# leaxer-ai/leaxer-qwen3-tts

Measured on AMD Instinct MI355X. Metric: real-time factor (24 kHz audio sec / wall sec), Qwen3-TTS-0.6B, higher is better.
Workload: dtype bf16 weights, fp32 activations/accumulate (codec decoder: fp16 hi/lo split operands, fp32 accumulate)

## Files before the change

### leaxer-qwen3-tts_amd/csrc/q3_codec.cpp

```cpp
#include <algorithm>
#include <cmath>
#include <cstdlib>
#include <cstring>
#include <unordered_map>
#include <vector>

#include "q3_engine.h"

namespace q3 {

struct PackedConv { const float* w = nullptr; const float* b = nullptr; int cin = 0, cout = 0, k = 0; };
struct SnakeP { const float *alpha = nullptr, *beta = nullptr; int C = 0; };

struct CodecW {
    struct Layer { const float *in_norm, *post_norm, *qkv, *o, *gate, *up, *down, *attn_scale, *mlp_scale; };
    std::vector<Layer> layers;
    const float *norm = nullptr, *code_embed = nullptr;
    struct Up { PackedConv tconv; const float *dw_w, *dw_b, *ln_w, *ln_b, *pw1_w, *pw1_b, *pw2_w, *pw2_b, *gamma; };
    std::vector<Up> up;
    PackedConv conv_in, conv_out;
    struct Res { SnakeP a1, a2; PackedConv c1, c2; };
    struct Block { SnakeP act; PackedConv tconv; Res res[3]; };
    std::vector<Block> blocks;
    SnakeP snake_out;
// ... 246 lines not shown
        auto take = [&](size_t nfloat) -> float* {
            const size_t bytes = (nfloat * sizeof(float) + 255) & ~(size_t)255;
            float* p = plan ? nullptr : (float*)(W.arena[lane] + off);
            off += bytes;
            return p;
        };
        const size_t kslab_floats = (size_t)32 * 128 * 4096;
        float* kslab = take(kslab_floats);
        auto conv = [&](ConvArgs a) {
            if (plan) return;
            a.slab = kslab; a.slab_floats = kslab_floats; a.batch = nbatch;
            const auto it = W.planes.find(a.W);
            if (it != W.planes.end()) { a.Wh = it->second.hi; a.Wl = it->second.lo; a.Whc = it->second.cm; a.w_scale_inv = it->second.scale_inv; a.w_lo_zero = it->second.lo_zero; }
            if (a.snake_alpha) { const auto sp = W.snake_pre.find(a.snake_alpha); if (sp != W.snake_pre.end()) a.snake_pre = sp->second; }
            if (a.mid_alpha) { const auto sp = W.snake_pre.find(a.mid_alpha); if (sp != W.snake_pre.end()) a.mid_pre = sp->second; }
            launch_conv(a, stream);
        };
        auto gemm = [&](const float* in, int T, int Cin, const float* Wm, const float* bias, int Cout, float* out) {
            ConvArgs a; a.in = in; a.T_in = T; a.C_in = Cin; a.out = out; a.T_out = T; a.C_out = Cout; a.W = Wm; a.bias = bias;
            return a;
        };
        float* h = take((size_t)F * CH);
        float* hn = take((size_t)F * CH);
        float* qkvb = take((size_t)F * 3 * CH);
        float* att = take((size_t)F * CH);
        float* ub = take((size_t)F * FF);
        float* gb = take((size_t)F * FF);
        float* kc = take((size_t)NH * P * HD);
        float* vc = take((size_t)NH * P * HD);
        if (!plan && !h_in) launch_code_embed_mean(W.code_embed, codes_dev, F, c.n_groups, c.cd_codebook, CH, h, stream);
        for (int l = 0; l < (h_in ? 0 : c.cd_layers); ++l) {
            const CodecW::Layer& L = W.layers[l];
            if (!plan) launch_rmsnorm_rows(h, L.in_norm, c.cd_rms_eps, F, CH, hn, stream);
// ... 35 lines not shown
        }
        const bool fp32_act = knob("Q3TTS_CONV_FP32_ACT") != nullptr || knob("Q3TTS_CONV_GENERIC_EPILOGUE") != nullptr;
        bool act_planes = !fp32_act && !W.planes.empty() && CH % 32 == 0 && W.planes.count(W.conv_in.w) && !W.snake_pre.empty();
        for (int i = 0, Cw = D; i <= c.cd_n_blocks; ++i, Cw /= 2) act_planes = act_planes && Cw % 96 == 0;
        for (const CodecW::Block& B : W.blocks) {
            act_planes = act_planes && W.planes.count(B.tconv.w);
            for (int u = 0; u < 3; ++u) act_planes = act_planes && W.planes.count(B.res[u].c1.w) && W.planes.count(B.res[u].c2.w);
        }
        float* x = take(nbz * Tc * D);
        float* sx = take(nbz * Tc * D);
        { ConvArgs a; a.in = cur; a.T_in = Tc; a.C_in = CH; a.out = x; a.T_out = Tc; a.C_out = D; a.W = W.conv_in.w; a.bias = W.conv_in.b; a.taps = 7;
          a.in_ustride = nbatch > 1 ? h_ustride : 0;
          a.out2 = sx; a.snake_alpha = W.blocks[0].act.alpha; a.snake_beta = W.blocks[0].act.beta; a.out2_planes = act_planes; conv(a); }
        int C = D;
        static const int dil[3] = { 1, 3, 9 };
        for (int i = 0; i < c.cd_n_blocks; ++i) {
            const CodecW::Block& B = W.blocks[i];
            const int r = c.cd_up_rates[i], Co = C / 2;
            int left = 0;
            const int To = tconv_out_len(c, Tc, 2 * r, r, &left);
            float* nx = take(nbz * To * Co);
            float* ns = take(nbz * To * Co);
            float* nt = take(nbz * To * Co);
            { ConvArgs a; a.in = sx; a.T_in = Tc; a.C_in = C; a.out = nx; a.T_out = To; a.C_out = Co; a.W = B.tconv.w; a.bias = B.tconv.b;
              a.taps = 2 * r; a.transposed = 1; a.stride = r; a.left = left; a.in_planes = act_planes;
              a.out2 = ns; a.snake_alpha = B.res[0].a1.alpha; a.snake_beta = B.res[0].a1.beta; a.out2_planes = act_planes; conv(a); }
            for (int u = 0; u < 3; ++u) {
                const CodecW::Res& R = B.res[u];
                const SnakeP nxt = u < 2 ? B.res[u + 1].a1 : (i + 1 < c.cd_n_blocks ? W.blocks[i + 1].act : W.snake_out);
                const bool nxt_planes = act_planes && !(u == 2 && i + 1 == c.cd_n_blocks);
                const auto p2 = W.planes.find(R.c2.w);
                if (Co == 96 && p2 != W.planes.end() && W.planes.count(R.c1.w) && !knob("Q3TTS_NO_FUSED_RES")) {
                    ConvArgs a; a.in = ns; a.T_in = To; a.C_in = Co; a.out = nx; a.T_out = To; a.C_out = Co; a.W = R.c1.w; a.bias = R.c1.b;
                    a.taps = 7; a.dil = dil[u]; a.mid_alpha = R.a2.alpha; a.mid_beta = R.a2.beta;
                    a.W2 = R.c2.w; a.W2h = p2->second.hi; a.W2l = p2->second.lo; a.W2fh = p2->second.fh; a.W2fl = p2->second.fl; a.w2_scale_inv = p2->second.scale_inv; a.w2_lo_zero = p2->second.lo_zero; a.bias2 = R.c2.b;
// ... 2 lines not shown
                    conv(a);
                    std::swap(ns, nt);
                    continue;
                }
                { ConvArgs a; a.in = ns; a.T_in = To; a.C_in = Co; a.out = nullptr; a.T_out = To; a.C_out = Co; a.W = R.c1.w; a.bias = R.c1.b;
                  a.taps = 7; a.dil = dil[u]; a.out2 = nt; a.snake_alpha = R.a2.alpha; a.snake_beta = R.a2.beta;
                  a.in_planes = act_planes; a.out2_planes = act_planes; conv(a); }
                { ConvArgs a; a.in = nt; a.T_in = To; a.C_in = Co; a.out = nx; a.T_out = To; a.C_out = Co; a.W = R.c2.w; a.bias = R.c2.b;
                  a.taps = 1; a.res = nx; a.out2 = ns; a.snake_alpha = nxt.alpha; a.snake_beta = nxt.beta;
                  a.in_planes = act_planes; a.out2_planes = nxt_planes; conv(a); }
            }
            x = nx; sx = ns; Tc = To; C = Co;
        }
        pcm = take(nbz * Tc);
        { ConvArgs a; a.in = sx; a.T_in = Tc; a.C_in = C; a.out = pcm; a.T_out = Tc; a.C_out = 1; a.W = W.conv_out.w; a.bias = W.conv_out.b;
          a.taps = 7; a.clamp = 1; conv(a); }
        if (!plan && nbatch > 1) { W.dbg_sx = sx; W.dbg_pcm = pcm; W.dbg_T = Tc; W.dbg_C = C; W.dbg_nb = nbatch; }
        n_pcm = Tc;
        if (plan && off > W.arena_bytes[lane]) {
            Q3_HIP_CHECK(hipStreamSynchronize(stream));
            if (W.arena[lane]) (void)hipFree(W.arena[lane]);
            W.arena[lane] = nullptr;
            Q3_HIP_CHECK(hipMalloc((void**)&W.arena[lane], off));
            W.arena_bytes[lane] = off;
        }
    }
    *pcm_dev = pcm;
    return n_pcm;
}


// ... 1128 lines not shown
```

### leaxer-qwen3-tts_amd/csrc/q3_codec_kernels.hip

```cpp
#include <cstdlib>
#include <type_traits>
#include <utility>

#include "q3_common.h"

namespace q3 {

typedef float f32x16 __attribute__((ext_vector_type(16)));

#ifdef Q3_SAMPLE_PROF
__device__ long long g_conv_prof[64];
void conv_prof_read(long long* out) { (void)hipMemcpyFromSymbol(out, HIP_SYMBOL(g_conv_prof), sizeof(long long) * 64); }
#ifndef Q3_CONV_PROF_SEL
#define Q3_CONV_PROF_SEL (a.taps == 1 && a.C_in == 3072 && a.C_out == 1024)
#endif
#ifndef Q3_CONV_PROF_WG
#define Q3_CONV_PROF_WG 0
#endif
#define CP_MARK_IF(k, lim) do { __builtin_amdgcn_sched_barrier(0); \
        if ((k) < (lim) && blockIdx.x == Q3_CONV_PROF_WG && blockIdx.y == 0 && blockIdx.z == 0 && threadIdx.x == 0 && (Q3_CONV_PROF_SEL)) g_conv_prof[k] = wall_clock64(); \
        __builtin_amdgcn_sched_barrier(0); } while (0)
#define CP_MARK(k) CP_MARK_IF(k, 64)
#define CP_MARK_L(k) CP_MARK_IF(k, 46)
#else
// ... 32 lines not shown
    int act, clamp;
    float* out2; const float* s2_alpha; const float* s2_beta;
    const bf16_t* Wh; const bf16_t* Wl;
    float acc_scale;
    int ksplit; float* slab;
    int xcd_map;
    int no_fast_epi;
    int peel_taps;
    int in_planes, out2_planes;
    const float* s2_pre; const float* s1_pre;
    int batch_tiles;
    size_t in_ustride;
    const bf16_t* W2h; const bf16_t* W2l; float acc_scale2; const float* bias2; const float* s1_alpha; const float* s1_beta;
    int wlo;
    const bf16_t* W2fh; const bf16_t* W2fl;
};

static __device__ __forceinline__ void conv_tile_ids(bool remap, int& bx, int& by, int& bz) {
    bx = blockIdx.x; by = blockIdx.y; bz = blockIdx.z;
    const int nx = gridDim.x, ny = gridDim.y, nyz = ny * gridDim.z;
    if (!remap || nyz == 1) return;
    const int L = bx + nx * (by + ny * bz), gsz = 8 * nyz, full = nx >> 3;
    int G = L / gsz, w = 8;
    if (G >= full) { G = full; w = nx & 7; }
    const int r = L - G * gsz;
    bx = G * 8 + r % w;
    const int yz = r / w;
    by = yz % ny; bz = yz / ny;
}

// ... 88 lines not shown

typedef _Float16 f16x8 __attribute__((ext_vector_type(8)));
typedef _Float16 f16x4 __attribute__((ext_vector_type(4)));
#define B3_LD 40

typedef _Float16 f16x2 __attribute__((ext_vector_type(2)));
typedef float f32x2 __attribute__((ext_vector_type(2)));
static __device__ __forceinline__ void split_f16x2(float a, float b, f16x2& hi, f16x2& lo) {
    const f32x2 c = { __builtin_amdgcn_fmed3f(a, -65504.f, 65504.f), __builtin_amdgcn_fmed3f(b, -65504.f, 65504.f) };
    hi = __builtin_convertvector(c, f16x2);
    const f32x2 back = __builtin_convertvector(hi, f32x2);
    const f32x2 r = { __builtin_amdgcn_fmed3f(a - back.x, -65504.f, 65504.f), __builtin_amdgcn_fmed3f(b - back.y, -65504.f, 65504.f) };
    lo = __builtin_convertvector(r, f16x2);
}
__device__ float g_conv_dump[2][64 * 4];
template <int NB, bool OUT, bool RES, int RH, bool O2P = false>
static __device__ __forceinline__ void split_epilogue_snake(const ConvKArgs& a, const f32x16 (&acc)[NB], float* stage, int mrow0, int co0w,
                                                            int lane, int phase, int NT) {
    constexpr int W = NB * 32, LDE = W + 8;
    const int c4 = lane & 31, rsel = lane >> 5;
    const int co = co0w + c4 * 4;
    const bool colok = c4 * 4 < W && co < a.C_out;
    const int coc = colok ? co : 0, lc = c4 * 4 < W ? c4 * 4 : 0;
    const int m0r = mrow0 + rsel;
    const int t0 = a.transposed ? m0r * a.stride + phase - a.left : m0r, tstep = a.transposed ? 2 * a.stride : 2;
    const int mlim = a.transposed ? a.T_in + NT - 1 : 0x7fffffff;
    auto row_ok = [&](int p) { const int t = t0 + p * tstep; return colok && t >= 0 && t < a.T_out && m0r + 2 * p < mlim; };
    auto row_off = [&](int p) -> size_t { return row_ok(p) ? (size_t)(t0 + p * tstep) * a.C_out + coc : (size_t)coc; };
    float4 resv[RH];
    auto load_res = [&](int slot0, int p0, int n) {
#pragma unroll
        for (int k = 0; k < n; ++k) resv[slot0 + k] = *reinterpret_cast<const float4*>(a.res + row_off(p0 + k));
    };
    if (RES) load_res(0, 0, RH);
    const float4 bias4 = *reinterpret_cast<const float4*>(a.bias + coc);
    const float4 ea4 = *reinterpret_cast<const float4*>(a.s2_pre + coc), ib4 = *reinterpret_cast<const float4*>(a.s2_pre + a.C_out + coc);
#pragma unroll
    for (int j = 0; j < NB; ++j)
#pragma unroll
        for (int reg = 0; reg < 16; ++reg) stage[((reg & 3) + 8 * (reg >> 2) + 4 * rsel) * LDE + j * 32 + c4] = acc[j][reg];
    const float ea[4] = { ea4.x, ea4.y, ea4.z, ea4.w }, ib[4] = { ib4.x, ib4.y, ib4.z, ib4.w };
    const float bs[4] = { bias4.x, bias4.y, bias4.z, bias4.w };
    float* const dump1 = &g_conv_dump[0][lane * 4];
    float* const dump2 = &g_conv_dump[1][lane * 4];
#pragma unroll
    for (int p = 0; p < 16; ++p) {
        const bool okp = row_ok(p);
        const size_t o = row_off(p);
        const float4 raw = *reinterpret_cast<const float4*>(&stage[(p * 2 + rsel) * LDE + lc]);
        float v[4] = { raw.x, raw.y, raw.z, raw.w }, s2[4];
        const float4 r4 = RES ? resv[p % RH] : make_float4(0.f, 0.f, 0.f, 0.f);
        const float rv[4] = { r4.x, r4.y, r4.z, r4.w };
#pragma unroll
        for (int e = 0; e < 4; ++e) {
            float x = v[e] * a.acc_scale + bs[e];
            if (RES) x = rv[e] + x;
            v[e] = x;
            s2[e] = x + ib[e] * sin_sq(x * ea[e]);
        }
        if (OUT) *reinterpret_cast<float4*>(okp ? a.out + o : dump1) = make_float4(v[0], v[1], v[2], v[3]);
        if (O2P) {
            f16x2 h01, h23, l01, l23;
            split_f16x2(s2[0], s2[1], h01, l01);
            split_f16x2(s2[2], s2[3], h23, l23);
            *reinterpret_cast<uint4*>(okp ? a.out2 + o : dump2) =
                make_uint4(__builtin_bit_cast(unsigned, h01), __builtin_bit_cast(unsigned, h23), __builtin_bit_cast(unsigned, l01), __builtin_bit_cast(unsigned, l23));
        } else
        *reinterpret_cast<float4*>(okp ? a.out2 + o : dump2) = make_float4(s2[0], s2[1], s2[2], s2[3]);
        if ((p & 3) == 3) {
            __builtin_amdgcn_sched_barrier(0);
            if (RES && RH == 8 && p < 8) load_res(p - 3, p + 5, 4);
            __builtin_amdgcn_sched_barrier(0);
        }
    }
}

template <int NB, int RH = 16>
static __device__ __forceinline__ void split_epilogue_block(const ConvKArgs& a, const f32x16 (&acc)[NB], float* stage, int mrow0, int co0w,
                                                            int lane, int phase, int NT) {
    if (a.out2 && a.s2_pre && a.bias && a.act == 0 && !a.mul && !a.res_scale && !a.no_fast_epi) {
        if (a.out2_planes) {
            if (a.res) { if (a.out) split_epilogue_snake<NB, true, true, RH, true>(a, acc, stage, mrow0, co0w, lane, phase, NT);
                         else split_epilogue_snake<NB, false, true, RH, true>(a, acc, stage, mrow0, co0w, lane, phase, NT); }
            else { if (a.out) split_epilogue_snake<NB, true, false, RH, true>(a, acc, stage, mrow0, co0w, lane, phase, NT);
                   else split_epilogue_snake<NB, false, false, RH, true>(a, acc, stage, mrow0, co0w, lane, phase, NT); }
            return;
        }
        if (a.res) { if (a.out) split_epilogue_snake<NB, true, true, RH>(a, acc, stage, mrow0, co0w, lane, phase, NT);
                     else split_epilogue_snake<NB, false, true, RH>(a, acc, stage, mrow0, co0w, lane, phase, NT); }
        else { if (a.out) split_epilogue_snake<NB, true, false, RH>(a, acc, stage, mrow0, co0w, lane, phase, NT);
               else split_epilogue_snake<NB, false, false, RH>(a, acc, stage, mrow0, co0w, lane, phase, NT); }
        return;
    }
    constexpr int W = NB * 32, LDE = W + 8;
// ... 61 lines not shown
                }
                if (okp) {
                    if (a.out) *reinterpret_cast<float4*>(a.out + o) = make_float4(v[0], v[1], v[2], v[3]);
                    if (OUT2) *reinterpret_cast<float4*>(a.out2 + o) = make_float4(s2[0], s2[1], s2[2], s2[3]);
                }
            }
#pragma unroll
            for (int k = 0; k < 4; ++k) { resv[k] = resn[k]; mulv[k] = muln[k]; }
        }
    };
    using I0 = std::integral_constant<int, 0>; using I1 = std::integral_constant<int, 1>; using I2 = std::integral_constant<int, 2>;
    if (a.out2) { if (a.act == 0) rows(I0{}, std::true_type{}); else if (a.act == 1) rows(I1{}, std::true_type{}); else rows(I2{}, std::true_type{}); }
    else { if (a.act == 0) rows(I0{}, std::false_type{}); else if (a.act == 1) rows(I1{}, std::false_type{}); else rows(I2{}, std::false_type{}); }
}

template <int MB, int NB, int WM, int WN, int PA, int KC = 32, int NBUF = 2, bool F2 = false, bool PEEL = false, bool APL = false, bool WLO = true>
__global__ __launch_bounds__(256) __attribute__((amdgpu_waves_per_eu((MB * NB <= 6 && KC == 32 ? 2 : 1), (MB * NB <= 6 && KC == 32 ? 2 : 1))))
void k_conv_split(ConvKArgs a0) {
    ConvKArgs a = a0;
    int bx, by, bz;
    conv_tile_ids(a.xcd_map != 0, bx, by, bz);
    bx = conv_batch_rebase(a, bx);
    constexpr int TM = WM * MB * 32, TN = WN * NB * 32, AROWS = PA * 32;
    constexpr int CB = KC / 32, SEG = KC / 8, LD = KC + 8;
    constexpr int BPL = WLO ? 2 : 1, PBT = TN * SEG * BPL;
    constexpr int PB = (PBT + 255) / 256;
    constexpr int A_BYTES = 2 * AROWS * LD * 2, B_BYTES = NBUF * 2 * TN * LD * 2;
    constexpr int E_BYTES = 4 * 32 * (NB * 32 + 8) * 4;
    constexpr int SM_BYTES = A_BYTES + B_BYTES > E_BYTES ? A_BYTES + B_BYTES : E_BYTES;
    __shared__ __attribute__((aligned(16))) unsigned char smem[SM_BYTES];
    _Float16 (*As)[AROWS][LD] = reinterpret_cast<_Float16 (*)[AROWS][LD]>(smem);
// ... 16 lines not shown
        for (int j = 0; j < NB; ++j) acc[i][j] = zero16;

    const int arow = tid >> 3, acol = (tid & 7) * 4;
    typedef unsigned u32x4 __attribute__((ext_vector_type(4)));
    typedef float f32x4v __attribute__((ext_vector_type(4)));
    f32x4v areg[PA][CB];
    u32x4 breg[PB];
    const char* const in_bytes = reinterpret_cast<const char*>(a.in);
    unsigned aoff[PA];
#pragma unroll
    for (int i = 0; i < PA; ++i) {
        const int src = m0 - halo + arow + 32 * i;
        const int sc = src < 0 ? 0 : (src < a.T_in ? src : a.T_in - 1);
        aoff[i] = ((unsigned)sc * (unsigned)a.C_in + (unsigned)acol) * 4u;
    }
    auto loadA = [&](int ci0) {
        const char* const base = in_bytes + (size_t)ci0 * 4;
#pragma unroll
        for (int i = 0; i < PA; ++i)
#pragma unroll
            for (int cb = 0; cb < CB; ++cb) areg[i][cb] = *reinterpret_cast<const f32x4v*>(base + cb * 128 + aoff[i]);
    };
    const char* const w_bytes = reinterpret_cast<const char*>(a.Wh);
    const unsigned w_lo = (unsigned)(reinterpret_cast<const char*>(a.Wl) - reinterpret_cast<const char*>(a.Wh));
    constexpr bool w_cm = KC == 32;
    const unsigned w_rowb = w_cm ? 64u : (unsigned)a.C_in * 2u;
    unsigned boff[PB];
#pragma unroll
    for (int i = 0; i < PB; ++i) {
        int idx = tid + 256 * i;
        if (PBT % 256 != 0 && idx >= PBT) idx -= PBT;
        const int plane = idx / (TN * SEG), rem = idx % (TN * SEG), brow = rem / SEG, bseg = rem % SEG;
        const int co = co0 + brow;
        const int cc = co < a.C_out ? co : a.C_out - 1;
        boff[i] = (plane ? w_lo : 0u) + (unsigned)cc * w_rowb + (unsigned)bseg * 16u;
    }
    auto loadB = [&](int ci0, int ti) {
        const int wtap = a.transposed ? phase + ti * a.stride : ti;
        const char* const base = w_bytes + (w_cm ? ((size_t)wtap * (a.C_in >> 5) + (ci0 >> 5)) * a.C_out * 64 : ((size_t)wtap * a.C_out * a.C_in + ci0) * 2);
#pragma unroll
        for (int i = 0; i < PB; ++i) breg[i] = *reinterpret_cast<const u32x4*>(base + boff[i]);
    };
    auto storeA = [&]() {
#pragma unroll
        for (int i = 0; i < PA; ++i) {
            const int src = m0 - halo + arow + 32 * i;
            const bool inr = src >= 0 && src < a.T_in;
#pragma unroll
            for (int cb = 0; cb < CB; ++cb) {
                const f32x4v r = areg[i][cb];
                const float4 v = make_float4(inr ? r.x : 0.f, inr ? r.y : 0.f, inr ? r.z : 0.f, inr ? r.w : 0.f);
                if (APL) {
                    *reinterpret_cast<uint2*>(&As[0][arow + 32 * i][cb * 32 + acol]) = make_uint2(__float_as_uint(v.x), __float_as_uint(v.y));
                    *reinterpret_cast<uint2*>(&As[1][arow + 32 * i][cb * 32 + acol]) = make_uint2(__float_as_uint(v.z), __float_as_uint(v.w));
                    continue;
                }
                f16x2 h01, h23, l01, l23;
                split_f16x2(v.x, v.y, h01, l01);
                split_f16x2(v.z, v.w, h23, l23);
                *reinterpret_cast<uint2*>(&As[0][arow + 32 * i][cb * 32 + acol]) = make_uint2(__builtin_bit_cast(unsigned, h01), __builtin_bit_cast(unsigned, h23));
                *reinterpret_cast<uint2*>(&As[1][arow + 32 * i][cb * 32 + acol]) = make_uint2(__builtin_bit_cast(unsigned, l01), __builtin_bit_cast(unsigned, l23));
            }
        }
    };
    auto storeB = [&](int buf) {
#pragma unroll
        for (int i = 0; i < PB; ++i) {
// ... 231 lines not shown
                const int kof = st * 16 + 8 * rsel;
                const f16x8 ah = *reinterpret_cast<const f16x8*>(&ts[col0 * TLD + kof]);
                const f16x8 al = *reinterpret_cast<const f16x8*>(&ts[(32 + col0) * TLD + kof]);
#pragma unroll
                for (int j = 0; j < NB; ++j) {
                    acc2[j] = __builtin_amdgcn_mfma_f32_32x32x16_f16(al, wbh[st & 1][j], acc2[j], 0, 0, 0);
                    if constexpr (WLO) acc2[j] = __builtin_amdgcn_mfma_f32_32x32x16_f16(ah, wbl[st & 1][j], acc2[j], 0, 0, 0);
                    acc2[j] = __builtin_amdgcn_mfma_f32_32x32x16_f16(ah, wbh[st & 1][j], acc2[j], 0, 0, 0);
                }
                __builtin_amdgcn_sched_barrier(0);
            }
            __builtin_amdgcn_fence(__ATOMIC_RELEASE, "wavefront");
            __builtin_amdgcn_wave_barrier();
            __builtin_amdgcn_fence(__ATOMIC_ACQUIRE, "wavefront");
            CP_MARK(50 + 4 * i);
            if (a.out2_planes) split_epilogue_snake<NB, true, true, 8, true>(a, acc2, stage, m0 + wm * MB * 32 + i * 32, co0, lane, 0, NT);
            else split_epilogue_snake<NB, true, true, 8>(a, acc2, stage, m0 + wm * MB * 32 + i * 32, co0, lane, 0, NT);
            __builtin_amdgcn_fence(__ATOMIC_RELEASE, "wavefront");
            __builtin_amdgcn_wave_barrier();
            __builtin_amdgcn_fence(__ATOMIC_ACQUIRE, "wavefront");
            CP_MARK(51 + 4 * i);
        };
        unit(std::integral_constant<int, 0>{});
        if constexpr (MB > 1) unit(std::integral_constant<int, MB - 1>{});
        static_assert(MB <= 2, "fused residual unit: at most two row blocks per wave");
        CP_MARK(63);
        return;
    }
    if constexpr (KC == 128) {
        if (ksp) {
            ConvKArgs b = a;
            b.out = a.slab + (size_t)bz * a.T_out * a.C_out;
            b.bias = nullptr; b.res = nullptr; b.res_scale = nullptr; b.mul = nullptr; b.out2 = nullptr; b.act = 0; b.acc_scale = 1.0f;
            split_epilogue_block<NB>(b, acc[0], stage, m0 + wm * MB * 32, co0 + wn * NB * 32, lane, 0, NT);
            if (MB > 1) split_epilogue_block<NB>(b, acc[MB - 1], stage, m0 + wm * MB * 32 + 32, co0 + wn * NB * 32, lane, 0, NT);
            return;
        }
    }
    CP_MARK(60);
    split_epilogue_block<NB>(a, acc[0], stage, m0 + wm * MB * 32, co0 + wn * NB * 32, lane, phase, NT);
    CP_MARK(61);
    if (MB > 1) split_epilogue_block<NB>(a, acc[MB - 1], stage, m0 + wm * MB * 32 + 32, co0 + wn * NB * 32, lane, phase, NT);
    CP_MARK(63);
}

__global__ __launch_bounds__(256) void k_conv_finish(ConvKArgs a) {
    const size_t n4 = (size_t)a.T_out * a.C_out / 4, i = (size_t)blockIdx.x * 256 + threadIdx.x;
    if (i >= n4) return;
    const size_t o = i * 4, plane = (size_t)a.T_out * a.C_out;
    const int co = (int)(o % a.C_out);
    float4 s4 = *reinterpret_cast<const float4*>(a.slab + o);
    for (int z = 1; z < a.ksplit; ++z) {
        const float4 p = *reinterpret_cast<const float4*>(a.slab + z * plane + o);
        s4.x += p.x; s4.y += p.y; s4.z += p.z; s4.w += p.w;
    }
    const float4 one4 = make_float4(1.f, 1.f, 1.f, 1.f), zero4 = make_float4(0.f, 0.f, 0.f, 0.f);
    const float4 b4 = a.bias ? *reinterpret_cast<const float4*>(a.bias + co) : zero4;
// ... 140 lines not shown
            x[p][c] = v.x; x[p][c + 1] = v.y; x[p][c + 2] = v.z; x[p][c + 3] = v.w;
        }
    }
    float w[MAXT][CPT];
#pragma unroll
    for (int tap = 0; tap < MAXT; ++tap) {
        const float* wr = a.W + (size_t)(tap < a.taps ? tap : 0) * a.C_in + s8 * CPT;
#pragma unroll
        for (int c = 0; c < CPT; c += 4) {
            const float4 v = *reinterpret_cast<const float4*>(wr + c);
            const bool on = tap < a.taps;
            w[tap][c] = on ? v.x : 0.f; w[tap][c + 1] = on ? v.y : 0.f; w[tap][c + 2] = on ? v.z : 0.f; w[tap][c + 3] = on ? v.w : 0.f;
        }
    }
    __builtin_amdgcn_sched_barrier(0);
    unsigned long long clk0 = 0, rt0 = 0;
    if constexpr (DUMP) {
        asm volatile("s_waitcnt vmcnt(0)" ::: "memory");
        clk0 = __builtin_amdgcn_s_memtime(); rt0 = __builtin_amdgcn_s_memrealtime();
    }
#pragma unroll
    for (int p = 0; p < NP; ++p) {
        const int src = t0 - halo + p * 32 + rl;
        const bool inr = src >= 0 && src < a.T_in;
        float d[MAXT];
#pragma unroll
        for (int tap = 0; tap < MAXT; ++tap) {
            float acc = 0.f;
#pragma unroll
            for (int c = 0; c < CPT; ++c) acc = fmaf(w[tap][c], x[p][c], acc);
// ... 54 lines not shown
    a.ksplit = 0; a.slab = nullptr; a.batch_tiles = 0;
    const bool no_xcd_map = knob("Q3TTS_CONV_NO_XCD_MAP") != nullptr;
    a.xcd_map = no_xcd_map ? 0 : 1;
    const bool no_fast_epi = knob("Q3TTS_CONV_GENERIC_EPILOGUE") != nullptr;
    a.no_fast_epi = no_fast_epi ? 1 : 0;
    const bool no_peel = knob("Q3TTS_CONV_NO_PEEL") != nullptr;
    a.peel_taps = no_peel ? 0 : 1;
    a.in_planes = c.in_planes ? 1 : 0; a.out2_planes = c.out2_planes ? 1 : 0;
    if (c.in_planes || c.out2_planes) {
        const bool split_ok = c.Wh && c.Wl && c.C_in % 32 == 0 && c.C_out >= 32 && c.C_out % 96 == 0 && !c.clamp;
        if (!split_ok || (c.out2_planes && !(c.out2 && c.snake_pre && c.bias && c.act == 0 && !c.mul && !c.res_scale && !no_fast_epi)))
            throw Error("conv: (hi, lo)-plane activations need a 96-multiple decoder conv on the split-precision path");
    }
    a.W2h = nullptr; a.W2l = nullptr; a.acc_scale2 = 1.0f; a.bias2 = nullptr; a.s1_alpha = nullptr; a.s1_beta = nullptr;
    a.W2fh = nullptr; a.W2fl = nullptr;
    auto use_cm = [&]() {
        if (c.Whc == nullptr || c.Wh == nullptr || c.Wl == nullptr) throw Error("conv: the 32-wide-chunk kernels need the chunk-major weight planes (ConvArgs::Whc)");
        a.Wl = c.Whc + (c.Wl - c.Wh); a.Wh = c.Whc;
    };
    a.in_ustride = c.in_ustride ? c.in_ustride : (size_t)c.T_in * c.C_in;
    const int nb = c.batch > 1 ? c.batch : 1;
    if (c.transposed && c.taps % c.stride != 0) throw Error("conv: transposed kernel must be a multiple of the stride");
    const int rows = c.transposed ? c.T_in + c.taps / c.stride - 1 : c.T_out;
    dim3 grid((rows + CT_M - 1) / CT_M, (c.C_out + CT_N - 1) / CT_N, c.transposed ? c.stride : 1);
    if (rows <= 0) return;
    if (c.C_out == 1 && !c.transposed && c.C_in == 96 && c.taps <= 8 && (c.taps - 1) * c.dil <= 64 && c.out && !c.out2 && !c.res && !c.mul &&
        !c.res_scale && c.act == 0 && !knob("Q3TTS_COUT1_LDS")) {
        const int to1 = CO1R_ROWS - (c.taps - 1) * c.dil, tiles = (c.T_out + to1 - 1) / to1;
        if (nb > 1) a.batch_tiles = tiles;
        const dim3 g1((unsigned)(tiles * nb));
        if (const char* v = knob("Q3TTS_COUT1_PACKED")) {
            if (const char* d = knob("Q3TTS_COUT1_DELAY_US")) hipLaunchKernelGGL(k_idle_us, dim3(1), dim3(64), 0, s, atoi(d));
            if (atoi(v) == 2 && nb > 1) {
                const size_t need = (size_t)tiles * nb * CO1R_ROWS * 8;
                if (need > g_cout1_dbg_floats) { Q3_HIP_CHECK(hipDeviceSynchronize()); if (g_cout1_dbg) (void)hipFree(g_cout1_dbg); g_cout1_dbg = nullptr; g_cout1_dbg_floats = 0; Q3_HIP_CHECK(hipMalloc((void**)&g_cout1_dbg, need * sizeof(float))); g_cout1_dbg_floats = need; }
                g_cout1_dbg_used = need;
                a.out2 = g_cout1_dbg;
                hipLaunchKernelGGL((k_conv_cout1_reg<12, true, true>), g1, dim3(256), 0, s, a);
            } else hipLaunchKernelGGL((k_conv_cout1_reg<12, true, false>), g1, dim3(256), 0, s, a);
            Q3_HIP_CHECK(hipGetLastError());
            return;
        }
        hipLaunchKernelGGL(k_conv_cout1_reg<12>, g1, dim3(256), 0, s, a);
        Q3_HIP_CHECK(hipGetLastError());
        return;
    }
    if (c.C_out == 1 && !c.transposed && c.C_in % 4 == 0 && c.out && !c.out2 && !c.res && !c.mul && !c.res_scale && c.act == 0) {
        const size_t lds = (size_t)(CO1_T + (c.taps - 1) * c.dil) * (c.C_in + 1) * sizeof(float);
        if (lds <= 60 * 1024) {
            const int tiles = (c.T_out + CO1_T - 1) / CO1_T;
            if (nb > 1) a.batch_tiles = tiles;
            hipLaunchKernelGGL(k_conv_cout1, dim3(tiles * nb), dim3(CO1_T), lds, s, a);
            Q3_HIP_CHECK(hipGetLastError());
            return;
        }
    }
    const int NTt = c.transposed ? c.taps / c.stride : c.taps;
    const int halo = c.transposed ? NTt - 1 : (c.taps - 1) * c.dil;
    if (c.Wh && c.Wl && (size_t)c.T_in * c.C_in * sizeof(float) >= ((size_t)1 << 32))
        throw Error("conv: one sequence's activation exceeds 4 GB (beyond ~5500 frames): decode it in chunks (q3tts_codec_decode_chunked_host)");
    if (c.Wh && c.Wl && !(c.Wl > c.Wh && (size_t)((const char*)c.Wl - (const char*)c.Wh) < ((size_t)1 << 31)))
        throw Error("conv: the lo weight plane must follow the hi plane within 2 GB (one allocation)");
    if (c.W2h != nullptr) {
        if (!(c.Wh && c.Wl && c.W2l && c.C_in == 96 && c.C_out == 96 && !c.transposed && halo <= 64 && c.mid_pre && c.snake_pre && c.bias2 && c.res && c.out && c.out2 && !c.res_scale && !c.clamp && c.act == 0 && !c.mul))
            throw Error("conv: fused residual unit needs 96 -> 96 channels on the split-precision path");
        a.acc_scale = c.w_scale_inv;
        a.W2h = c.W2h; a.W2l = c.W2l; a.acc_scale2 = c.w2_scale_inv; a.bias2 = c.bias2; a.s1_alpha = c.mid_alpha; a.s1_beta = c.mid_beta; a.s1_pre = c.mid_pre;
        if (c.W2fh && c.W2fl && !knob("Q3TTS_CONV_W2_ROWMAJOR")) { a.W2fh = c.W2fh; a.W2fl = c.W2fl; }
        use_cm();
        const int extra = (halo + 31) / 32, tiles = (rows + 255) / 256;
        if (nb > 1) a.batch_tiles = tiles;
        const dim3 g((unsigned)(tiles * nb), 1, 1);
#define Q3_FUSED(PA_, PEEL_, APL_) Q3_CS(g, s, a, 2, 3, 4, 1, PA_, 32, 2, true, PEEL_, APL_)
        const bool peel = a.peel_taps && (a.wlo ? c.taps >= 3 : c.taps == 7), wide = extra > 1;
        if (a.in_planes) { if (peel) { if (wide) Q3_FUSED(10, true, true); else Q3_FUSED(9, true, true); } else { if (wide) Q3_FUSED(10, false, true); else Q3_FUSED(9, false, true); } }
        else { if (peel) { if (wide) Q3_FUSED(10, true, false); else Q3_FUSED(9, true, false); } else { if (wide) Q3_FUSED(10, false, false); else Q3_FUSED(9, false, false); } }
#undef Q3_FUSED
        Q3_HIP_CHECK(hipGetLastError());
        return;
    }
    if (c.Wh && c.Wl && c.C_in % 32 == 0 && c.C_out >= 32 && c.C_out % 4 == 0 && halo <= 64 && !c.clamp) {
        a.acc_scale = c.w_scale_inv;
        const int extra = (halo + 31) / 32, z = c.transposed ? c.stride : 1;
        const bool n96 = c.C_out % 96 == 0;
        const int ntile = n96 ? c.C_out / 96 : (c.C_out + 127) / 128;
        const long n_big = (long)((rows + 255) / 256) * ntile * z * nb, n_thin = (long)((rows + 127) / 128) * ntile * z * nb;
        auto bgrid = [&](int tiles, int gy, int gz) { if (nb > 1) a.batch_tiles = tiles; return dim3((unsigned)(tiles * nb), (unsigned)gy, (unsigned)gz); };
        const bool deep = NTt * c.C_in > 512;
        if (n_thin < 256) {
            const dim3 g = bgrid((rows + 63) / 64, (c.C_out + 127) / 128, z);
            int ks = 1;
            if (nb == 1 && c.taps == 1 && !c.transposed && c.C_in % 128 == 0 && c.C_in >= 512 && c.slab) {
                const int nch = c.C_in / 128;
                for (ks = 1; ks < nch; ++ks)
                    if (nch % ks == 0 && (long)g.x * g.y * ks >= 256) break;
                while (ks > 1 && (nch % ks != 0 || (size_t)ks * c.T_out * c.C_out > c.slab_floats)) --ks;
            }
            if (ks > 1) {
                a.ksplit = ks; a.slab = c.slab;
                if (a.in_planes) Q3_CS(dim3(g.x, g.y, ks), s, a, 2, 1, 1, 4, 2, 128, 1, false, false, true);
                else Q3_CS(dim3(g.x, g.y, ks), s, a, 2, 1, 1, 4, 2, 128, 1, false, false, false);
                const size_t n4 = (size_t)c.T_out * c.C_out / 4;
                hipLaunchKernelGGL(k_conv_finish, dim3((unsigned)((n4 + 255) / 256)), dim3(256), 0, s, a);
                Q3_HIP_CHECK(hipGetLastError());
                return;
// ... 351 lines not shown
```

### leaxer-qwen3-tts_amd/csrc/q3_common.h

```cpp
#pragma once
#include <hip/hip_runtime.h>
#include <stdint.h>
#include <string>

#include "../../include/q3tts.h"

typedef uint16_t bf16_t;

#define Q3_HIP_CHECK(expr)                                                                         \
    do {                                                                                           \
        hipError_t _e = (expr);                                                                    \
        if (_e != hipSuccess) throw q3::Error(std::string(#expr) + ": " + hipGetErrorString(_e));  \
    } while (0)

namespace q3 {

struct Error {
    std::string msg;
    explicit Error(std::string m) : msg(std::move(m)) {}
};

const char* knob(const char* name);
struct KnobScope {
    bool on = false;
// ... 250 lines not shown
    float w_scale_inv = 1.0f;
    bool w_lo_zero = false, w2_lo_zero = false;
    const float* bias = nullptr;
    int taps = 1, dil = 1;
    int transposed = 0, stride = 1, left = 0;
    int act = 0;
    const float* mul = nullptr;
    const float* res_scale = nullptr;
    const float* res = nullptr;
    int clamp = 0;
    float* out2 = nullptr;
    const float* snake_alpha = nullptr;
    const float* snake_beta = nullptr;
    bool in_planes = false, out2_planes = false;
    const float* snake_pre = nullptr;
    float* slab = nullptr; size_t slab_floats = 0;
    const float* W2 = nullptr; const bf16_t* W2h = nullptr; const bf16_t* W2l = nullptr; float w2_scale_inv = 1.0f;
    const bf16_t* Whc = nullptr; const bf16_t* W2fh = nullptr; const bf16_t* W2fl = nullptr;
    const float* bias2 = nullptr; const float* mid_alpha = nullptr; const float* mid_beta = nullptr; const float* mid_pre = nullptr;
    int batch = 1;
    size_t in_ustride = 0;
};
void launch_conv(const ConvArgs& a, hipStream_t s);
void cout1_debug_buffer(const float** p, size_t* n);
void launch_split_planes(const float* w, bf16_t* hi, bf16_t* lo, size_t n, float scale, hipStream_t s);
void launch_snake_pre(const float* alpha, const float* beta, float* pre , int C, hipStream_t s);
void launch_repack_planes_cm(const bf16_t* planes , bf16_t* out , int taps, int cout, int cin, size_t plane_elems, hipStream_t s);
void launch_pack_w2_frags(const bf16_t* plane , bf16_t* out , int C, hipStream_t s);
void launch_absmax(const float* w, size_t n, unsigned* out, hipStream_t s);
void launch_or_mag16(const bf16_t* p, size_t n, unsigned* out , hipStream_t s);
// ... 171 lines not shown
```

Measured before the change: 42.69.

## Apply SnakeBeta at input staging in last decoder block instead of writing second outputs

For the final 96-channel decoder block, the transposed conv and fused residual units now write only the plain fp32 activation. The SnakeBeta activation is recomputed from precomputed constants when each consumer stages its input, including the 96->1 output conv. This removes the extra snake-activated output buffer (out2/nt) written and re-read per unit at the highest time resolution. The cost is that the sin is recomputed per tap-load in staging, and several knob combinations are now rejected.

```diff
diff --git a/leaxer-qwen3-tts_amd/csrc/q3_codec.cpp b/leaxer-qwen3-tts_amd/csrc/q3_codec.cpp
--- a/leaxer-qwen3-tts_amd/csrc/q3_codec.cpp
+++ b/leaxer-qwen3-tts_amd/csrc/q3_codec.cpp
@@ -284,9 +284,10 @@
             if (it != W.planes.end()) { a.Wh = it->second.hi; a.Wl = it->second.lo; a.Whc = it->second.cm; a.w_scale_inv = it->second.scale_inv; a.w_lo_zero = it->second.lo_zero; }
             if (a.snake_alpha) { const auto sp = W.snake_pre.find(a.snake_alpha); if (sp != W.snake_pre.end()) a.snake_pre = sp->second; }
             if (a.mid_alpha) { const auto sp = W.snake_pre.find(a.mid_alpha); if (sp != W.snake_pre.end()) a.mid_pre = sp->second; }
+            if (a.in_snake_alpha) { const auto sp = W.snake_pre.find(a.in_snake_alpha); if (sp != W.snake_pre.end()) a.in_snake_pre = sp->second; }
             launch_conv(a, stream);
         };
-        auto gemm = [&](const float* in, int T, int Cin, const float* Wm, const float* bias, int Cout, float* out) {
+        auto gemm =[&](const float* in, int T, int Cin, const float* Wm, const float* bias, int Cout, float* out) {
             ConvArgs a; a.in = in; a.T_in = T; a.C_in = Cin; a.out = out; a.T_out = T; a.C_out = Cout; a.W = Wm; a.bias = bias;
             return a;
         };
@@ -352,11 +353,34 @@
           a.out2 = sx; a.snake_alpha = W.blocks[0].act.alpha; a.snake_beta = W.blocks[0].act.beta; a.out2_planes = act_planes; conv(a); }
         int C = D;
         static const int dil[3] = { 1, 3, 9 };
+        const float* sx_snake = nullptr;
         for (int i = 0; i < c.cd_n_blocks; ++i) {
             const CodecW::Block& B = W.blocks[i];
             const int r = c.cd_up_rates[i], Co = C / 2;
             int left = 0;
             const int To = tconv_out_len(c, Tc, 2 * r, r, &left);
+            bool stage_snake = act_planes && Co == 96 && i + 1 == c.cd_n_blocks && !knob("Q3TTS_NO_FUSED_RES") &&
+                               !knob("Q3TTS_COUT1_LDS") && !knob("Q3TTS_COUT1_PACKED");
+            if (const char* v = knob("Q3TTS_CONV_STAGE_SNAKE")) stage_snake = stage_snake && atoi(v) != 0;
+            if (stage_snake) {
+                float* xa = take(nbz * To * Co);
+                float* xb = take(nbz * To * Co);
+                { ConvArgs a; a.in = sx; a.T_in = Tc; a.C_in = C; a.out = xa; a.T_out = To; a.C_out = Co; a.W = B.tconv.w; a.bias = B.tconv.b;
+                  a.taps = 2 * r; a.transposed = 1; a.stride = r; a.left = left; a.in_planes = act_planes; a.out_plain = true; conv(a); }
+                for (int u = 0; u < 3; ++u) {
+                    const CodecW::Res& R = B.res[u];
+                    const auto p2 = W.planes.find(R.c2.w);
+                    if (p2 == W.planes.end()) throw Error("codec: the fused residual unit needs the split-precision planes of its 1x1 conv");
+                    ConvArgs a; a.in = xa; a.T_in = To; a.C_in = Co; a.out = xb; a.T_out = To; a.C_out = Co; a.W = R.c1.w; a.bias = R.c1.b;
+                    a.taps = 7; a.dil = dil[u]; a.mid_alpha = R.a2.alpha; a.mid_beta = R.a2.beta; a.in_snake_alpha = R.a1.alpha;
+                    a.W2 = R.c2.w; a.W2h = p2->second.hi; a.W2l = p2->second.lo; a.W2fh = p2->second.fh; a.W2fl = p2->second.fl; a.w2_scale_inv = p2->second.scale_inv; a.w2_lo_zero = p2->second.lo_zero; a.bias2 = R.c2.b;
+                    a.res = xa;
+                    conv(a);
+                    std::swap(xa, xb);
+                }
+                x = xa; sx = xa; sx_snake = W.snake_out.alpha; Tc = To; C = Co;
+                continue;
+            }
             float* nx = take(nbz * To * Co);
             float* ns = take(nbz * To * Co);
             float* nt = take(nbz * To * Co);
@@ -389,7 +413,7 @@
         }
         pcm = take(nbz * Tc);
         { ConvArgs a; a.in = sx; a.T_in = Tc; a.C_in = C; a.out = pcm; a.T_out = Tc; a.C_out = 1; a.W = W.conv_out.w; a.bias = W.conv_out.b;
-          a.taps = 7; a.clamp = 1; conv(a); }
+          a.taps = 7; a.clamp = 1; a.in_snake_alpha = sx_snake; conv(a); }
         if (!plan && nbatch > 1) { W.dbg_sx = sx; W.dbg_pcm = pcm; W.dbg_T = Tc; W.dbg_C = C; W.dbg_nb = nbatch; }
         n_pcm = Tc;
         if (plan && off > W.arena_bytes[lane]) {
diff --git a/leaxer-qwen3-tts_amd/csrc/q3_codec_kernels.hip b/leaxer-qwen3-tts_amd/csrc/q3_codec_kernels.hip
--- a/leaxer-qwen3-tts_amd/csrc/q3_codec_kernels.hip
+++ b/leaxer-qwen3-tts_amd/csrc/q3_codec_kernels.hip
@@ -70,6 +70,7 @@
     const bf16_t* W2h; const bf16_t* W2l; float acc_scale2; const float* bias2; const float* s1_alpha; const float* s1_beta;
     int wlo;
     const bf16_t* W2fh; const bf16_t* W2fl;
+    const float* sin_pre; int out_plain;
 };
 
 static __device__ __forceinline__ void conv_tile_ids(bool remap, int& bx, int& by, int& bz) {
@@ -188,7 +189,7 @@
     lo = __builtin_convertvector(r, f16x2);
 }
 __device__ float g_conv_dump[2][64 * 4];
-template <int NB, bool OUT, bool RES, int RH, bool O2P = false>
+template <int NB, bool OUT, bool RES, int RH, bool O2P = false, bool O2 = true>
 static __device__ __forceinline__ void split_epilogue_snake(const ConvKArgs& a, const f32x16 (&acc)[NB], float* stage, int mrow0, int co0w,
                                                             int lane, int phase, int NT) {
     constexpr int W = NB * 32, LDE = W + 8;
@@ -208,7 +209,8 @@
     };
     if (RES) load_res(0, 0, RH);
     const float4 bias4 = *reinterpret_cast<const float4*>(a.bias + coc);
-    const float4 ea4 = *reinterpret_cast<const float4*>(a.s2_pre + coc), ib4 = *reinterpret_cast<const float4*>(a.s2_pre + a.C_out + coc);
+    const float4 zero4 = make_float4(0.f, 0.f, 0.f, 0.f);
+    const float4 ea4 = O2 ? *reinterpret_cast<const float4*>(a.s2_pre + coc) : zero4, ib4 = O2 ? *reinterpret_cast<const float4*>(a.s2_pre + a.C_out + coc) : zero4;
 #pragma unroll
     for (int j = 0; j < NB; ++j)
 #pragma unroll
@@ -230,10 +232,11 @@
             float x = v[e] * a.acc_scale + bs[e];
             if (RES) x = rv[e] + x;
             v[e] = x;
-            s2[e] = x + ib[e] * sin_sq(x * ea[e]);
+            if (O2) s2[e] = x + ib[e] * sin_sq(x * ea[e]);
         }
         if (OUT) *reinterpret_cast<float4*>(okp ? a.out + o : dump1) = make_float4(v[0], v[1], v[2], v[3]);
-        if (O2P) {
+        if (!O2) { }
+        else if (O2P) {
             f16x2 h01, h23, l01, l23;
             split_f16x2(s2[0], s2[1], h01, l01);
             split_f16x2(s2[2], s2[3], h23, l23);
@@ -249,9 +252,12 @@
     }
 }
 
-template <int NB, int RH = 16>
+template <int NB, int RH = 16, bool PLAIN = false>
 static __device__ __forceinline__ void split_epilogue_block(const ConvKArgs& a, const f32x16 (&acc)[NB], float* stage, int mrow0, int co0w,
                                                             int lane, int phase, int NT) {
+    if constexpr (PLAIN) {
+        if (a.out_plain) { split_epilogue_snake<NB, true, false, RH, false, false>(a, acc, stage, mrow0, co0w, lane, phase, NT); return; }
+    }
     if (a.out2 && a.s2_pre && a.bias && a.act == 0 && !a.mul && !a.res_scale && !a.no_fast_epi) {
         if (a.out2_planes) {
             if (a.res) { if (a.out) split_epilogue_snake<NB, true, true, RH, true>(a, acc, stage, mrow0, co0w, lane, phase, NT);
@@ -343,7 +349,7 @@
     else { if (a.act == 0) rows(I0{}, std::false_type{}); else if (a.act == 1) rows(I1{}, std::false_type{}); else rows(I2{}, std::false_type{}); }
 }
 
-template <int MB, int NB, int WM, int WN, int PA, int KC = 32, int NBUF = 2, bool F2 = false, bool PEEL = false, bool APL = false, bool WLO = true>
+template <int MB, int NB, int WM, int WN, int PA, int KC = 32, int NBUF = 2, bool F2 = false, bool PEEL = false, int APL = 0, bool WLO = true>
 __global__ __launch_bounds__(256) __attribute__((amdgpu_waves_per_eu((MB * NB <= 6 && KC == 32 ? 2 : 1), (MB * NB <= 6 && KC == 32 ? 2 : 1))))
 void k_conv_split(ConvKArgs a0) {
     ConvKArgs a = a0;
@@ -390,12 +396,18 @@
         const int sc = src < 0 ? 0 : (src < a.T_in ? src : a.T_in - 1);
         aoff[i] = ((unsigned)sc * (unsigned)a.C_in + (unsigned)acol) * 4u;
     }
+    static_assert(APL != 2 || (F2 && KC == 32), "SnakeBeta at staging: the fused residual unit (one column tile)");
+    f32x4v sreg[APL == 2 ? 2 : 1];
     auto loadA = [&](int ci0) {
         const char* const base = in_bytes + (size_t)ci0 * 4;
 #pragma unroll
         for (int i = 0; i < PA; ++i)
 #pragma unroll
             for (int cb = 0; cb < CB; ++cb) areg[i][cb] = *reinterpret_cast<const f32x4v*>(base + cb * 128 + aoff[i]);
+        if constexpr (APL == 2) {
+            sreg[0] = *reinterpret_cast<const f32x4v*>(a.sin_pre + ci0 + acol);
+            sreg[1] = *reinterpret_cast<const f32x4v*>(a.sin_pre + a.C_in + ci0 + acol);
+        }
     };
     const char* const w_bytes = reinterpret_cast<const char*>(a.Wh);
     const unsigned w_lo = (unsigned)(reinterpret_cast<const char*>(a.Wl) - reinterpret_cast<const char*>(a.Wh));
@@ -424,9 +436,13 @@
             const bool inr = src >= 0 && src < a.T_in;
 #pragma unroll
             for (int cb = 0; cb < CB; ++cb) {
-                const f32x4v r = areg[i][cb];
+                f32x4v r = areg[i][cb];
+                if constexpr (APL == 2) {
+#pragma unroll
+                    for (int e = 0; e < 4; ++e) r[e] = r[e] + sreg[1][e] * sin_sq(r[e] * sreg[0][e]);
+                }
                 const float4 v = make_float4(inr ? r.x : 0.f, inr ? r.y : 0.f, inr ? r.z : 0.f, inr ? r.w : 0.f);
-                if (APL) {
+                if (APL == 1) {
                     *reinterpret_cast<uint2*>(&As[0][arow + 32 * i][cb * 32 + acol]) = make_uint2(__float_as_uint(v.x), __float_as_uint(v.y));
                     *reinterpret_cast<uint2*>(&As[1][arow + 32 * i][cb * 32 + acol]) = make_uint2(__float_as_uint(v.z), __float_as_uint(v.w));
                     continue;
@@ -688,7 +704,8 @@
             __builtin_amdgcn_wave_barrier();
             __builtin_amdgcn_fence(__ATOMIC_ACQUIRE, "wavefront");
             CP_MARK(50 + 4 * i);
-            if (a.out2_planes) split_epilogue_snake<NB, true, true, 8, true>(a, acc2, stage, m0 + wm * MB * 32 + i * 32, co0, lane, 0, NT);
+            if constexpr (APL == 2) split_epilogue_snake<NB, true, true, 8, false, false>(a, acc2, stage, m0 + wm * MB * 32 + i * 32, co0, lane, 0, NT);
+            else if (a.out2_planes) split_epilogue_snake<NB, true, true, 8, true>(a, acc2, stage, m0 + wm * MB * 32 + i * 32, co0, lane, 0, NT);
             else split_epilogue_snake<NB, true, true, 8>(a, acc2, stage, m0 + wm * MB * 32 + i * 32, co0, lane, 0, NT);
             __builtin_amdgcn_fence(__ATOMIC_RELEASE, "wavefront");
             __builtin_amdgcn_wave_barrier();
@@ -712,9 +729,10 @@
         }
     }
     CP_MARK(60);
-    split_epilogue_block<NB>(a, acc[0], stage, m0 + wm * MB * 32, co0 + wn * NB * 32, lane, phase, NT);
+    constexpr bool PLAIN = KC == 32 && !F2 && (NB == 3 || NB == 1);
+    split_epilogue_block<NB, 16, PLAIN>(a, acc[0], stage, m0 + wm * MB * 32, co0 + wn * NB * 32, lane, phase, NT);
     CP_MARK(61);
-    if (MB > 1) split_epilogue_block<NB>(a, acc[MB - 1], stage, m0 + wm * MB * 32 + 32, co0 + wn * NB * 32, lane, phase, NT);
+    if (MB > 1) split_epilogue_block<NB, 16, PLAIN>(a, acc[MB - 1], stage, m0 + wm * MB * 32 + 32, co0 + wn * NB * 32, lane, phase, NT);
     CP_MARK(63);
 }
 
@@ -885,6 +903,22 @@
         }
     }
     __builtin_amdgcn_sched_barrier(0);
+    if constexpr (!PACKED) {
+        if (a.sin_pre) {
+            float ea[CPT], ib[CPT];
+#pragma unroll
+            for (int c = 0; c < CPT; c += 4) {
+                const float4 e4 = *reinterpret_cast<const float4*>(a.sin_pre + s8 * CPT + c), i4 = *reinterpret_cast<const float4*>(a.sin_pre + a.C_in + s8 * CPT + c);
+                ea[c] = e4.x; ea[c + 1] = e4.y; ea[c + 2] = e4.z; ea[c + 3] = e4.w;
+                ib[c] = i4.x; ib[c + 1] = i4.y; ib[c + 2] = i4.z; ib[c + 3] = i4.w;
+            }
+#pragma unroll
+            for (int p = 0; p < NP; ++p)
+#pragma unroll
+                for (int c = 0; c < CPT; ++c) x[p][c] = x[p][c] + ib[c] * sin_sq(x[p][c] * ea[c]);
+        }
+        __builtin_amdgcn_sched_barrier(0);
+    }
     unsigned long long clk0 = 0, rt0 = 0;
     if constexpr (DUMP) {
         asm volatile("s_waitcnt vmcnt(0)" ::: "memory");
@@ -969,6 +1003,11 @@
     }
     a.W2h = nullptr; a.W2l = nullptr; a.acc_scale2 = 1.0f; a.bias2 = nullptr; a.s1_alpha = nullptr; a.s1_beta = nullptr;
     a.W2fh = nullptr; a.W2fl = nullptr;
+    a.sin_pre = c.in_snake_pre; a.out_plain = c.out_plain ? 1 : 0;
+    if (c.in_snake_alpha && !c.in_snake_pre) throw Error("conv: SnakeBeta at staging needs the precomputed constants (ConvArgs::in_snake_pre)");
+    if (c.in_snake_pre && (c.in_planes || c.C_in != 96 || c.transposed)) throw Error("conv: SnakeBeta at staging is built for the 96-channel block's fp32 rows");
+    if (c.out_plain && !(c.Wh && c.Wl && c.C_in % 32 == 0 && c.C_out == 96 && c.out && !c.out2 && c.bias && !c.res && c.act == 0 && !c.mul && !c.res_scale && !c.clamp && !c.W2h))
+        throw Error("conv: out_plain is the 96-wide decoder conv's epilogue (bias only, no second output)");
     auto use_cm = [&]() {
         if (c.Whc == nullptr || c.Wh == nullptr || c.Wl == nullptr) throw Error("conv: the 32-wide-chunk kernels need the chunk-major weight planes (ConvArgs::Whc)");
         a.Wl = c.Whc + (c.Wl - c.Wh); a.Wh = c.Whc;
@@ -985,6 +1024,7 @@
         if (nb > 1) a.batch_tiles = tiles;
         const dim3 g1((unsigned)(tiles * nb));
         if (const char* v = knob("Q3TTS_COUT1_PACKED")) {
+            if (c.in_snake_pre) throw Error("conv: Q3TTS_COUT1_PACKED reads an fp32 SnakeBeta buffer: set Q3TTS_CONV_STAGE_SNAKE=0 with it");
             if (const char* d = knob("Q3TTS_COUT1_DELAY_US")) hipLaunchKernelGGL(k_idle_us, dim3(1), dim3(64), 0, s, atoi(d));
             if (atoi(v) == 2 && nb > 1) {
                 const size_t need = (size_t)tiles * nb * CO1R_ROWS * 8;
@@ -1000,6 +1040,7 @@
         Q3_HIP_CHECK(hipGetLastError());
         return;
     }
+    if (c.in_snake_pre && c.W2h == nullptr) throw Error("conv: SnakeBeta at staging exists in the fused 96-channel unit and the 96 -> 1 register kernel only");
     if (c.C_out == 1 && !c.transposed && c.C_in % 4 == 0 && c.out && !c.out2 && !c.res && !c.mul && !c.res_scale && c.act == 0) {
         const size_t lds = (size_t)(CO1_T + (c.taps - 1) * c.dil) * (c.C_in + 1) * sizeof(float);
         if (lds <= 60 * 1024) {
@@ -1017,7 +1058,8 @@
     if (c.Wh && c.Wl && !(c.Wl > c.Wh && (size_t)((const char*)c.Wl - (const char*)c.Wh) < ((size_t)1 << 31)))
         throw Error("conv: the lo weight plane must follow the hi plane within 2 GB (one allocation)");
     if (c.W2h != nullptr) {
-        if (!(c.Wh && c.Wl && c.W2l && c.C_in == 96 && c.C_out == 96 && !c.transposed && halo <= 64 && c.mid_pre && c.snake_pre && c.bias2 && c.res && c.out && c.out2 && !c.res_scale && !c.clamp && c.act == 0 && !c.mul))
+        const bool outs_ok = c.in_snake_pre ? (!c.out2 && c.res == c.in && c.out != c.in) : (c.out2 && c.snake_pre);
+        if (!(c.Wh && c.Wl && c.W2l && c.C_in == 96 && c.C_out == 96 && !c.transposed && halo <= 64 && c.mid_pre && outs_ok && c.bias2 && c.res && c.out && !c.res_scale && !c.clamp && c.act == 0 && !c.mul))
             throw Error("conv: fused residual unit needs 96 -> 96 channels on the split-precision path");
         a.acc_scale = c.w_scale_inv;
         a.W2h = c.W2h; a.W2l = c.W2l; a.acc_scale2 = c.w2_scale_inv; a.bias2 = c.bias2; a.s1_alpha = c.mid_alpha; a.s1_beta = c.mid_beta; a.s1_pre = c.mid_pre;
@@ -1028,7 +1070,8 @@
         const dim3 g((unsigned)(tiles * nb), 1, 1);
 #define Q3_FUSED(PA_, PEEL_, APL_) Q3_CS(g, s, a, 2, 3, 4, 1, PA_, 32, 2, true, PEEL_, APL_)
         const bool peel = a.peel_taps && (a.wlo ? c.taps >= 3 : c.taps == 7), wide = extra > 1;
-        if (a.in_planes) { if (peel) { if (wide) Q3_FUSED(10, true, true); else Q3_FUSED(9, true, true); } else { if (wide) Q3_FUSED(10, false, true); else Q3_FUSED(9, false, true); } }
+        if (a.sin_pre) { if (peel) { if (wide) Q3_FUSED(10, true, 2); else Q3_FUSED(9, true, 2); } else { if (wide) Q3_FUSED(10, false, 2); else Q3_FUSED(9, false, 2); } }
+        else if (a.in_planes) { if (peel) { if (wide) Q3_FUSED(10, true, true); else Q3_FUSED(9, true, true); } else { if (wide) Q3_FUSED(10, false, true); else Q3_FUSED(9, false, true); } }
         else { if (peel) { if (wide) Q3_FUSED(10, true, false); else Q3_FUSED(9, true, false); } else { if (wide) Q3_FUSED(10, false, false); else Q3_FUSED(9, false, false); } }
 #undef Q3_FUSED
         Q3_HIP_CHECK(hipGetLastError());
@@ -1044,6 +1087,7 @@
         const bool deep = NTt * c.C_in > 512;
         if (n_thin < 256) {
             const dim3 g = bgrid((rows + 63) / 64, (c.C_out + 127) / 128, z);
+            if (c.out_plain && c.C_in % 128 == 0) throw Error("conv: out_plain is not built into the 128-wide-chunk kernels");
             int ks = 1;
             if (nb == 1 && c.taps == 1 && !c.transposed && c.C_in % 128 == 0 && c.C_in >= 512 && c.slab) {
                 const int nch = c.C_in / 128;
diff --git a/leaxer-qwen3-tts_amd/csrc/q3_common.h b/leaxer-qwen3-tts_amd/csrc/q3_common.h
--- a/leaxer-qwen3-tts_amd/csrc/q3_common.h
+++ b/leaxer-qwen3-tts_amd/csrc/q3_common.h
@@ -288,6 +288,8 @@
     const float* snake_beta = nullptr;
     bool in_planes = false, out2_planes = false;
     const float* snake_pre = nullptr;
+    const float* in_snake_alpha = nullptr; const float* in_snake_pre = nullptr;
+    bool out_plain = false;
     float* slab = nullptr; size_t slab_floats = 0;
     const float* W2 = nullptr; const bf16_t* W2h = nullptr; const bf16_t* W2l = nullptr; float w2_scale_inv = 1.0f;
     const bf16_t* Whc = nullptr; const bf16_t* W2fh = nullptr; const bf16_t* W2fl = nullptr;
```

Measured after the change: 42.27. About the same (-1.0%).
